# paninski-lab/deepgraphpose

Hardware: AMD Instinct MI355X
Metric: frames_per_sec (higher is better)
Workload: dtype f32

## Files before the change

### deepgraphpose_amd/csrc/dgp_chain.hip

```cpp
#include "dgp_internal.h"
#include "dgp_device.h"

#include <cstdio>
#include <cstdlib>
#include <type_traits>

namespace dgp {

typedef float floatx4 __attribute__((ext_vector_type(4)));
typedef __attribute__((address_space(3))) void lds_void;

__device__ __forceinline__ floatx4 mma16(const uint4& a, const uint4& b, floatx4 c) {
    return __builtin_amdgcn_mfma_f32_16x16x32_f16(__builtin_bit_cast(half8, a), __builtin_bit_cast(half8, b), c, 0, 0, 0);
}
__device__ __forceinline__ uint4 ld16nt(__amdgpu_buffer_rsrc_t r, unsigned voff, int soff) {
    return __builtin_bit_cast(uint4, __builtin_amdgcn_raw_buffer_load_b128(r, (int)voff, soff, 2));
}
__device__ __forceinline__ void st16nt(__amdgpu_buffer_rsrc_t r, const uint4& v, unsigned voff, int soff) {
    __builtin_amdgcn_raw_buffer_store_b128(__builtin_bit_cast(u32x4, v), r, (int)voff, soff, 2);
}
__device__ __forceinline__ uint4 ld16(__amdgpu_buffer_rsrc_t r, unsigned voff, int soff) {
    return __builtin_bit_cast(uint4, __builtin_amdgcn_raw_buffer_load_b128(r, (int)voff, soff, 0));
}
__device__ __forceinline__ void st16(__amdgpu_buffer_rsrc_t r, const uint4& v, unsigned voff, int soff) {
    __builtin_amdgcn_raw_buffer_store_b128(__builtin_bit_cast(u32x4, v), r, (int)voff, soff, 0);
}

#ifdef DGP_DIAG
__device__ unsigned long long g_unit_diag[16];
#define UD_STAMP(x)                                                                     \
    do {                                                                                \
        __builtin_amdgcn_sched_barrier(0);                                              \
        asm volatile("s_memtime %0\n\ts_waitcnt lgkmcnt(0)" : "=s"(x)::"memory");       \
        __builtin_amdgcn_sched_barrier(0);                                              \
    } while (0)
#define UD_PARAM , unsigned long long (&ud)[12]
#define UD_ARG , ud
#else
#define UD_STAMP(x)
#define UD_PARAM
#define UD_ARG
#endif

template <int RES, int RB, bool H1 = false>
__device__ __forceinline__ void chain_fetch_res(const ChainArgs& p, uint4 (&res)[RB][2], const unsigned (&roff)[RB],
                                                const __amdgpu_buffer_rsrc_t rs_s2, int jp) {
    if constexpr (RES != 0) {
#pragma unroll
        for (int rb = 0; rb < RB; ++rb) {
            if constexpr (H1) {
                res[rb][0] = (p.nt & 1) ? ld16nt(rs_s2, roff[rb], jp * 64) : ld16(rs_s2, roff[rb], jp * 64);
            } else if (p.nt & 1) {
                res[rb][0] = ld16nt(rs_s2, roff[rb], jp * 128);
                res[rb][1] = ld16nt(rs_s2, roff[rb], jp * 128 + 16);
            } else {
                res[rb][0] = ld16(rs_s2, roff[rb], jp * 128);
                res[rb][1] = ld16(rs_s2, roff[rb], jp * 128 + 16);
            }
        }
    }
}
template <int RES, int RB, int PD, bool H1 = false>
__device__ __forceinline__ void chain_prefetch(const ChainArgs& p, uint4 (&res)[PD][RB][2], const unsigned (&roff)[RB],
                                               const __amdgpu_buffer_rsrc_t rs_s2) {
#pragma unroll
    for (int u = 0; u < PD - 1; ++u) chain_fetch_res<RES, RB, H1>(p, res[u], roff, rs_s2, u);
}

template <int C, int C1, int CIN2, int RES, int RB, int NS, int PD, int CHUNK, int WR, bool H1 = false>
__device__ __forceinline__ void chain_tail(const ChainArgs& p, const uint4* ring, int& slot, const uint4 (&ph)[RB][(C + CIN2) / 32],
                                           const uint4 (&pl)[RB][(C + CIN2) / 32], const unsigned (&xoff)[RB], const unsigned (&roff)[RB],
                                           const unsigned (&r1off)[RB], const unsigned long long (&xkeep)[RB], const bool xwave,
                                           const __amdgpu_buffer_rsrc_t rs_s2, const __amdgpu_buffer_rsrc_t rs_xo,
                                           const __amdgpu_buffer_rsrc_t rs_r1, float& amax_x, float& amax_r1, const int lane,
                                           uint4 (&res)[PD][RB][2] UD_PARAM) {
#ifdef DGP_DIAG
    unsigned long long c0 = 0, c1 = 0, c2 = 0, c3 = 0, c4 = 0;
#endif
    constexpr int C4 = 4 * C, KS1 = (C + CIN2) / 32, NJP = C4 / 32, NCB = C1 / 16;
    constexpr int PL = H1 ? 1 : 2;
    constexpr int F1 = KS1 * 2 * PL, F2 = NCB * PL;
    static_assert(WR >= 2 && WR % 2 == 0, "weight fragments in flight: pairs share the ring");
    static_assert(NJP % PD == 0 && PD >= 2, "chunk loop is unrolled PD times");
    const int g = lane >> 4;
    floatx4 a2[RB][NCB];
#pragma unroll
    for (int rb = 0; rb < RB; ++rb)
#pragma unroll
        for (int cb = 0; cb < NCB; ++cb) a2[rb][cb] = floatx4{0.f, 0.f, 0.f, 0.f};
    auto fetch_res = [&](int jp, int buf) { chain_fetch_res<RES, RB, H1>(p, res[buf], roff, rs_s2, jp); };
    constexpr int CB = H1 ? 64 : 128;
    for (int jp0 = 0; jp0 < NJP; jp0 += PD) {
#pragma unroll
        for (int u = 0; u < PD; ++u) {
            const int jp = jp0 + u;
            if (jp + PD - 1 < NJP) fetch_res(jp + PD - 1, (u + PD - 1) % PD);
            UD_STAMP(c0);
            const uint4* Wc = ring + slot * (CHUNK / 16);
            const uint4* W = Wc + lane;
            floatx4 a1[RB][2];
#pragma unroll
            for (int rb = 0; rb < RB; ++rb) { a1[rb][0] = floatx4{0.f, 0.f, 0.f, 0.f}; a1[rb][1] = floatx4{0.f, 0.f, 0.f, 0.f}; }
            uint4 wq[WR];
#pragma unroll
            for (int f = 0; f < WR && f < F1 + F2; ++f) wq[f] = W[f * 64];
            __builtin_amdgcn_sched_barrier(0);
#pragma unroll
            for (int s = 0; s < KS1; ++s)
#pragma unroll
                for (int b = 0; b < 2; ++b) {
                    const int f0 = (s * 2 + b) * PL;
                    const uint4 wh = wq[f0 % WR], wl = wq[(f0 + PL - 1) % WR];
                    if constexpr (!H1) {
#pragma unroll
                    for (int rb = 0; rb < RB; ++rb) a1[rb][b] = mma16(wl, ph[rb][s], a1[rb][b]);
#pragma unroll
                    for (int rb = 0; rb < RB; ++rb) a1[rb][b] = mma16(wh, pl[rb][s], a1[rb][b]);
                    }
#pragma unroll
                    for (int rb = 0; rb < RB; ++rb) a1[rb][b] = mma16(wh, ph[rb][s], a1[rb][b]);
                    __builtin_amdgcn_sched_barrier(0);
                    if (f0 + WR < F1 + F2) wq[f0 % WR] = W[(f0 + WR) * 64];
                    if (PL == 2 && f0 + 1 + WR < F1 + F2) wq[(f0 + 1) % WR] = W[(f0 + 1 + WR) * 64];
                    __builtin_amdgcn_sched_barrier(0);
                }
            UD_STAMP(c1);
            const float4 sa = __builtin_bit_cast(float4, Wc[(F1 + F2) * 64 + 2 * g]), sb = __builtin_bit_cast(float4, Wc[(F1 + F2) * 64 + 2 * g + 1]);
            const float4 ba = __builtin_bit_cast(float4, Wc[(F1 + F2) * 64 + 8 + 2 * g]), bb = __builtin_bit_cast(float4, Wc[(F1 + F2) * 64 + 8 + 2 * g + 1]);
            const float sc[8] = {sa.x * p.post1, sa.y * p.post1, sa.z * p.post1, sa.w * p.post1,
                                 sb.x * p.post1, sb.y * p.post1, sb.z * p.post1, sb.w * p.post1};
            const float bi[8] = {ba.x, ba.y, ba.z, ba.w, bb.x, bb.y, bb.z, bb.w};
            uint4 xh[RB], xl[RB];
#pragma unroll
            for (int rb = 0; rb < RB; ++rb) {
                float o[8], r[8] = {0.f, 0.f, 0.f, 0.f, 0.f, 0.f, 0.f, 0.f};
                if constexpr (RES != 0) {
                    if constexpr (H1) h1_unpack8(res[u][rb][0], p.res_inv_scale, r);
                    else h2_unpack8(res[u][rb][0], res[u][rb][1], p.res_inv_scale, r);
                }
#pragma unroll
                for (int k = 0; k < 8; ++k) {
                    o[k] = a1[rb][k >> 2][k & 3] * sc[k] + bi[k] + r[k];
                    o[k] = fmaxf(o[k], 0.f);
                }
                if constexpr (H1) { xh[rb] = h1_pack8(o, p.xout_scale); xl[rb] = xh[rb]; }
                else h2_pack8(o, p.xout_scale, xh[rb], xl[rb]);
                if (xwave) {
                    const unsigned so = __builtin_amdgcn_inverse_ballot_w64(xkeep[rb]) ? xoff[rb] : OOB;
                    if (p.nt & 2) {
                        st16nt(rs_xo, xh[rb], so, jp * CB);
                        if constexpr (!H1) st16nt(rs_xo, xl[rb], so, jp * CB + 16);
                    } else {
                        st16(rs_xo, xh[rb], so, jp * CB);
                        if constexpr (!H1) st16(rs_xo, xl[rb], so, jp * CB + 16);
                    }
                }
                if (xoff[rb] != OOB) {
#pragma unroll
                    for (int k = 0; k < 8; ++k) amax_x = fmaxf(amax_x, o[k]);
                }
            }
            UD_STAMP(c2);
            __builtin_amdgcn_sched_barrier(0);
#pragma unroll
            for (int cb = 0; cb < NCB; ++cb) {
                const int f0 = F1 + cb * PL;
                const uint4 wh = wq[f0 % WR], wl = wq[(f0 + PL - 1) % WR];
                if constexpr (!H1) {
#pragma unroll
                for (int rb = 0; rb < RB; ++rb) a2[rb][cb] = mma16(wl, xh[rb], a2[rb][cb]);
#pragma unroll
                for (int rb = 0; rb < RB; ++rb) a2[rb][cb] = mma16(wh, xl[rb], a2[rb][cb]);
                }
#pragma unroll
                for (int rb = 0; rb < RB; ++rb) a2[rb][cb] = mma16(wh, xh[rb], a2[rb][cb]);
                __builtin_amdgcn_sched_barrier(0);
                if (f0 + WR < F1 + F2) wq[f0 % WR] = W[(f0 + WR) * 64];
                if (PL == 2 && f0 + 1 + WR < F1 + F2) wq[(f0 + 1) % WR] = W[(f0 + 1 + WR) * 64];
                __builtin_amdgcn_sched_barrier(0);
            }
            slot = slot + 1 == NS ? 0 : slot + 1;
            UD_STAMP(c3);
            asm volatile("s_waitcnt lgkmcnt(0)" ::: "memory");
            __builtin_amdgcn_s_barrier();
            UD_STAMP(c4);
#ifdef DGP_DIAG
            ud[4] += c1 - c0; ud[5] += c2 - c1; ud[6] += c3 - c2; ud[7] += c4 - c3;
#endif
        }
    }
    UD_STAMP(c0);
#pragma unroll
    for (int q = 0; q < NCB / 2; ++q) {
        const float4 s0 = *reinterpret_cast<const float4*>(p.sc1 + 32 * q + 8 * g), s1 = *reinterpret_cast<const float4*>(p.sc1 + 32 * q + 8 * g + 4);
        const float4 b0 = *reinterpret_cast<const float4*>(p.bi1 + 32 * q + 8 * g), b1 = *reinterpret_cast<const float4*>(p.bi1 + 32 * q + 8 * g + 4);
        const float sc[8] = {s0.x * p.post2, s0.y * p.post2, s0.z * p.post2, s0.w * p.post2,
                             s1.x * p.post2, s1.y * p.post2, s1.z * p.post2, s1.w * p.post2};
        const float bi[8] = {b0.x, b0.y, b0.z, b0.w, b1.x, b1.y, b1.z, b1.w};
#pragma unroll
        for (int rb = 0; rb < RB; ++rb) {
            float o[8];
#pragma unroll
            for (int k = 0; k < 8; ++k) o[k] = fmaxf(a2[rb][2 * q + (k >> 2)][k & 3] * sc[k] + bi[k], 0.f);
            if constexpr (H1) {
                st16(rs_r1, h1_pack8(o, p.r1_scale), r1off[rb], q * CB);
            } else {
            uint4 hi, lo;
            h2_pack8(o, p.r1_scale, hi, lo);
            st16(rs_r1, hi, r1off[rb], q * 128);
            st16(rs_r1, lo, r1off[rb], q * 128 + 16);
            }
            if (r1off[rb] != OOB) {
#pragma unroll
                for (int k = 0; k < 8; ++k) amax_r1 = fmaxf(amax_r1, o[k]);
            }
        }
    }
    UD_STAMP(c1);
#ifdef DGP_DIAG
    ud[8] += c1 - c0;
#endif
}

template <int C, int C1, int CIN2, int RES, int RB, int NCW, int NLW, int NS, int PD, int WR, bool H1 = false>
__global__ __launch_bounds__(64 * (NCW + NLW)) void chain_kernel(const ChainArgs p) {
    constexpr int C4 = 4 * C;
    constexpr int EB = H1 ? 2 : 4;
    constexpr int KSA = C / 32, KSB = CIN2 / 32, KS1 = KSA + KSB;
    constexpr int NJP = C4 / 32;
    constexpr int NCB = C1 / 16;
    constexpr int PL = H1 ? 1 : 2;
    constexpr int F1 = KS1 * 2 * PL, F2 = NCB * PL, NF = F1 + F2 + 1;
    constexpr int CHUNK = NF * 1024;
    constexpr int TILE = 16 * RB * NCW;
    static_assert(NJP % PD == 0 && PD >= 2, "chunk loop is unrolled PD times");
    static_assert(RES == 0 || CIN2 == 0, "residual or K-concatenated shortcut, not both");
    static_assert(NS == 2 || NS == 3, "ring protocols of the loader below");
    extern __shared__ __attribute__((aligned(16))) char smem[];
    const int lane = threadIdx.x & 63;
    const int wave = __builtin_amdgcn_readfirstlane(threadIdx.x >> 6);
    const int my_tiles = (p.ntiles - (int)blockIdx.x + (int)gridDim.x - 1) / (int)gridDim.x;
    const int total = my_tiles * NJP;

    if (wave >= NCW) {
        const int lw = wave - NCW;
        const __amdgpu_buffer_rsrc_t rs_w = __builtin_amdgcn_make_buffer_rsrc(const_cast<void*>(p.wfrag), 0, (int)p.w_bytes, 0x00020000);
        int jp = 0, slot = 0;
        auto run = [&](auto niw) {
            constexpr int NIW = decltype(niw)::value;
            auto issue = [&]() {
                char* dst = smem + slot * CHUNK;
                const int gbase = jp * CHUNK;
#pragma unroll
                for (int i = 0; i < NIW; ++i) {
                    const int f = lw + i * NLW;
                    __builtin_amdgcn_raw_ptr_buffer_load_lds(rs_w, (lds_void*)(dst + f * 1024), 16, lane * 16, gbase + f * 1024, 0, 0);
                }
                jp = jp + 1 == NJP ? 0 : jp + 1;
                slot = slot + 1 == NS ? 0 : slot + 1;
            };
            if constexpr (NS == 3) {
                if (total > 0) issue();
                if (total > 1) { issue(); asm volatile("s_waitcnt vmcnt(%0)" ::"n"(NIW) : "memory"); }
                else asm volatile("s_waitcnt vmcnt(0)" ::: "memory");
                __builtin_amdgcn_s_barrier();
                for (int it = 0; it < total; ++it) {
                    if (it + 2 < total) { issue(); asm volatile("s_waitcnt vmcnt(%0)" ::"n"(NIW) : "memory"); }
                    else asm volatile("s_waitcnt vmcnt(0)" ::: "memory");
                    __builtin_amdgcn_s_barrier();
                }
            } else {
                if (total > 0) issue();
                asm volatile("s_waitcnt vmcnt(0)" ::: "memory");
                __builtin_amdgcn_s_barrier();
                for (int it = 0; it < total; ++it) {
                    if (it + 1 < total) issue();
                    asm volatile("s_waitcnt vmcnt(0)" ::: "memory");
                    __builtin_amdgcn_s_barrier();
                }
            }
        };
        constexpr int NI_HI = (NF + NLW - 1) / NLW, NI_LO = NF / NLW;
        if (lw < NF % NLW || NI_HI == NI_LO) run(std::integral_constant<int, NI_HI>());
        else run(std::integral_constant<int, NI_LO>());
        return;
    }

    const int l15 = lane & 15, g = lane >> 4;
    const __amdgpu_buffer_rsrc_t rs_r2 = __builtin_amdgcn_make_buffer_rsrc(const_cast<void*>(p.r2), 0, (int)p.r2_bytes, 0x00020000);
    const __amdgpu_buffer_rsrc_t rs_s2 = __builtin_amdgcn_make_buffer_rsrc(const_cast<void*>(p.src2 ? p.src2 : p.r2), 0,
                                                                            p.src2 ? (int)p.src2_bytes : 0, 0x00020000);
    const __amdgpu_buffer_rsrc_t rs_xo = __builtin_amdgcn_make_buffer_rsrc(p.xout, 0, (int)p.xout_bytes, 0x00020000);
    const __amdgpu_buffer_rsrc_t rs_r1 = __builtin_amdgcn_make_buffer_rsrc(p.r1out, 0, (int)p.r1_bytes, 0x00020000);
    const uint4* ring = reinterpret_cast<const uint4*>(smem);
    int slot = 0;
    float amax_x = 0.f, amax_r1 = 0.f;
    __builtin_amdgcn_s_barrier();
    for (int t = blockIdx.x; t < p.ntiles; t += gridDim.x) {
        unsigned xoff[RB], roff[RB], r1off[RB];
        unsigned long long xkeep[RB];
#pragma unroll
        for (int rb = 0; rb < RB; ++rb) xkeep[rb] = ~0ull;
        if (p.xkeep == 2) {
            unsigned HoWo = (unsigned)p.HoWo, Wo = (unsigned)p.Wo;
            asm volatile("" : "+s"(HoWo), "+s"(Wo));
#pragma unroll
            for (int rb = 0; rb < RB; ++rb) {
                const unsigned m = (unsigned)(t * TILE + (wave * RB + rb) * 16 + l15);
                const unsigned rem = m % HoWo, ho = rem / Wo, wo = rem - ho * Wo;
                xkeep[rb] = __builtin_amdgcn_ballot_w64(((ho | wo) & 1) == 0);
            }
        }
        uint4 ph[RB][KS1], pl[RB][KS1];
#pragma unroll
        for (int rb = 0; rb < RB; ++rb) {
            const int m = t * TILE + (wave * RB + rb) * 16 + l15;
            const bool ok = m < p.M;
            xoff[rb] = ok ? (unsigned)m * (unsigned)(C4 * EB) + (unsigned)(g * 8 * EB) : OOB;
            r1off[rb] = ok ? (unsigned)m * (unsigned)(C1 * EB) + (unsigned)(g * 8 * EB) : OOB;
            if (RES == 2) {
                const int n = m / p.HoWo, rem = m - n * p.HoWo, ho = rem / p.Wo, wo = rem - ho * p.Wo;
                roff[rb] = ok ? (unsigned)((n * p.res_H + 2 * ho) * p.res_W + 2 * wo) * (unsigned)(C4 * EB) + (unsigned)(g * 8 * EB) : OOB;
            } else roff[rb] = xoff[rb];
            const unsigned aoff = ok ? (unsigned)m * (unsigned)(C * EB) + (unsigned)(g * 8 * EB) : OOB;
#pragma unroll
            for (int s = 0; s < KSA; ++s) {
                ph[rb][s] = ld16(rs_r2, aoff, s * 32 * EB);
                if constexpr (H1) pl[rb][s] = ph[rb][s]; else pl[rb][s] = ld16(rs_r2, aoff, s * 128 + 16);
            }
            if constexpr (KSB > 0) {
                const unsigned boff = ok ? (unsigned)m * (unsigned)(CIN2 * EB) + (unsigned)(g * 8 * EB) : OOB;
#pragma unroll
                for (int s = 0; s < KSB; ++s) {
                    ph[rb][KSA + s] = ld16(rs_s2, boff, s * 32 * EB);
                    if constexpr (H1) pl[rb][KSA + s] = ph[rb][KSA + s]; else pl[rb][KSA + s] = ld16(rs_s2, boff, s * 128 + 16);
                }
            }
        }
        uint4 res[PD][RB][2];
        chain_prefetch<RES, RB, PD, H1>(p, res, roff, rs_s2);
#ifdef DGP_DIAG
        unsigned long long ud[12] = {0};
#endif
        chain_tail<C, C1, CIN2, RES, RB, NS, PD, CHUNK, WR, H1>(p, ring, slot, ph, pl, xoff, roff, r1off, xkeep, true, rs_s2, rs_xo, rs_r1, amax_x, amax_r1, lane, res UD_ARG);
#ifdef DGP_DIAG
        if (wave == 0 && lane == 0) {
            for (int i = 4; i < 9; ++i) atomicAdd(&g_unit_diag[i], ud[i]);
            atomicAdd(&g_unit_diag[9], 1ull);
        }
#endif
    }
    if (p.xout_absmax) track_absmax(p.xout_absmax, amax_x, lane, (int)(blockIdx.x * 8u + (unsigned)wave));
    if (p.r1_absmax) track_absmax(p.r1_absmax, amax_r1, lane, (int)(blockIdx.x * 8u + (unsigned)wave) + 97);
}

template <int C, int C1, int CIN2, int RES, int NCW, int NLW, int PD, int WR, int HWV = 1, bool H1 = false>
__global__ __launch_bounds__(64 * (NCW + NLW + HWV)) void unit_kernel(const ChainArgs p) {
    constexpr int NS = 3;
    constexpr int TH = NCW, TW = 16, HW = TW + 2, HPIX = (TH + 2) * HW;
    constexpr int EB = H1 ? 2 : 4;
    constexpr int PIXB = C * EB;
    constexpr int PPI = 1024 / PIXB;
    static_assert(C == 64, "one pixel of R1 = 16 (H1: 8) slots of 16 bytes (the bank swizzle)");
    constexpr int NHI = (HPIX * PIXB + 1023) / 1024;
    constexpr int HALO_BYTES = NHI * 1024;
    static_assert(NLW == 1 || NLW == 2 || NLW == 4, "one, two or four weight-loader waves");
    static_assert(HWV == 0 || HWV == 1, "at most one halo wave");
    constexpr int NHW = HWV ? 1 : NLW;
    constexpr int C4 = 4 * C, KS1 = (C + CIN2) / 32, NJP = C4 / 32, NCB = C1 / 16;
    constexpr int PL = H1 ? 1 : 2;
    constexpr int NFJ = (KS1 * 2 + NCB) * PL + 1;
    constexpr int KS2 = C / 32, NCB2 = C / 16, NF2 = KS2 * NCB2 * PL + 1;
    constexpr int NFMAX = NFJ > NF2 ? NFJ : NF2, CHUNK = NFMAX * 1024;
    constexpr int STEPS = 9 + NJP;
    constexpr int HSTEPS = HWV ? NJP - 1 : NJP;
    constexpr int HPP = (NHI + HSTEPS - 1) / HSTEPS;
    extern __shared__ __attribute__((aligned(16))) char smem[];
    char* halo = smem;
    char* ringb = smem + HALO_BYTES;
    const int lane = threadIdx.x & 63;
    const int wave = __builtin_amdgcn_readfirstlane(threadIdx.x >> 6);
    const int G = (int)gridDim.x, b = (int)blockIdx.x;
    const int vwg = (G & 7) == 0 ? (b & 7) * (G >> 3) + (b >> 3) : b;
    const int my_tiles = vwg < p.ntiles ? (p.ntiles - vwg + G - 1) / G : 0;
    const int total = my_tiles * STEPS;
    const int tpf = p.TY * p.TX;

    if (wave >= NCW) {
        auto halo_issue = [&](int tile, int i0, int i1, int hl) {
            const __amdgpu_buffer_rsrc_t rs_in = __builtin_amdgcn_make_buffer_rsrc(const_cast<void*>(p.r1in), 0, (int)p.r1in_bytes, 0x00020000);
            const int f = tile / tpf, rem = tile - f * tpf, ty = rem / p.TX, tx = rem - ty * p.TX;
            for (int i = i0 + hl; i < i1; i += NHW) {
                const int hp = PPI * i + (H1 ? (lane >> 3) : (lane >> 4));
                const int hy = (hp * 57) >> 10, hx = hp - HW * hy;
                const int gy = ty * TH - 1 + hy, gx = tx * TW - 1 + hx;
                const bool ok = hp < HPIX && (unsigned)gy < (unsigned)p.H && (unsigned)gx < (unsigned)p.W;
                const unsigned cell = H1 ? (unsigned)((lane & 7) ^ ((hp >> 1) & 7)) : (unsigned)((lane & 15) ^ (hp & 15));
                const unsigned off = ok ? (unsigned)((f * p.H + gy) * p.W + gx) * (unsigned)PIXB + (cell << 4) : OOB;
                __builtin_amdgcn_raw_ptr_buffer_load_lds(rs_in, (lds_void*)(halo + i * 1024), 16, (int)off, 0, 0, 0);
            }
        };
        auto halo_step = [&](int cur_st, int tile, int hl) {
            if (cur_st >= 9 && tile + G < p.ntiles) {
                const int i0 = (cur_st - 9) * HPP, i1 = i0 + HPP < NHI ? i0 + HPP : NHI;
                halo_issue(tile + G, i0, i1, hl);
            }
        };
        const int lw_rt = wave - NCW;
        if (HWV && lw_rt == NLW) {
            if (total > 0) halo_issue(vwg, 0, NHI, 0);
            asm volatile("s_waitcnt vmcnt(0)" ::: "memory");
            __builtin_amdgcn_s_barrier();
            int cur_st = 0, tile = vwg;
            for (int it = 0; it < total; ++it) {
                halo_step(cur_st, tile, 0);
                if (cur_st == STEPS - 1) asm volatile("s_waitcnt vmcnt(0)" ::: "memory");
                __builtin_amdgcn_s_barrier();
                if (++cur_st == STEPS) { cur_st = 0; tile += G; }
            }
            return;
        }
        auto loader = [&](auto lw_c) {
        constexpr int lw = decltype(lw_c)::value;
        const __amdgpu_buffer_rsrc_t rs_w = __builtin_amdgcn_make_buffer_rsrc(const_cast<void*>(p.wfrag), 0, (int)p.w_bytes, 0x00020000);
        int st = 0, slot = 0;
        constexpr int N2 = lw < NF2 % NLW ? (NF2 + NLW - 1) / NLW : NF2 / NLW, NJ = lw < NFJ % NLW ? (NFJ + NLW - 1) / NLW : NFJ / NLW;
        auto issue = [&]() {
            char* dst = ringb + slot * CHUNK;
            const int st2 = st, stj = st - 9;
            if (st < 9) {
#pragma unroll
                for (int k = 0; k < N2; ++k)
                    __builtin_amdgcn_raw_ptr_buffer_load_lds(rs_w, (lds_void*)(dst + (lw + k * NLW) * 1024), 16, lane * 16, st2 * (NF2 * 1024) + (lw + k * NLW) * 1024, 0, 0);
            } else {
#pragma unroll
                for (int k = 0; k < NJ; ++k)
                    __builtin_amdgcn_raw_ptr_buffer_load_lds(rs_w, (lds_void*)(dst + (lw + k * NLW) * 1024), 16, lane * 16,
                                                             9 * (NF2 * 1024) + stj * (NFJ * 1024) + (lw + k * NLW) * 1024, 0, 0);
            }
            const bool was_conv2 = st < 9;
            st = st + 1 == STEPS ? 0 : st + 1;
            slot = slot + 1 == NS ? 0 : slot + 1;
            return was_conv2;
        };
        auto wait_all_but_newest = [&](bool conv2_chunk) {
            if (conv2_chunk) asm volatile("s_waitcnt vmcnt(%0)" ::"n"(N2) : "memory");
            else asm volatile("s_waitcnt vmcnt(%0)" ::"n"(NJ) : "memory");
        };
        if (total > 0) {
            if (!HWV) halo_issue(vwg, 0, NHI, lw);
            issue();
            wait_all_but_newest(issue());
        }
        __builtin_amdgcn_s_barrier();
        int cur_st = 0, tile = vwg;
#ifdef DGP_DIAG
        unsigned long long l0 = 0, l1 = 0, l2 = 0, l3 = 0, ul[3] = {0, 0, 0}, ul3 = 0;
#endif
        for (int it = 0; it < total; ++it) {
            UD_STAMP(l0);
            if (!HWV) halo_step(cur_st, tile, lw);
#ifdef DGP_DIAG
            bool c2_ = false;
            if (it + 2 < total) c2_ = issue();
            UD_STAMP(l1);
            if (it + 2 < total) wait_all_but_newest(c2_);
            else asm volatile("s_waitcnt vmcnt(0)" ::: "memory");
            UD_STAMP(l2);
#else
            if (it + 2 < total) wait_all_but_newest(issue());
            else asm volatile("s_waitcnt vmcnt(0)" ::: "memory");
#endif
            __builtin_amdgcn_s_barrier();
            UD_STAMP(l3);
#ifdef DGP_DIAG
            if (cur_st < 9) ul[0] += l1 - l0; else ul3 += l1 - l0;
            ul[1] += l2 - l1; ul[2] += l3 - l2;
#endif
            if (++cur_st == STEPS) { cur_st = 0; tile += G; }
        }
#ifdef DGP_DIAG
        if (lw == 0 && lane == 0) {
            atomicAdd(&g_unit_diag[12], ul[0]); atomicAdd(&g_unit_diag[13], ul[1]); atomicAdd(&g_unit_diag[14], ul[2]); atomicAdd(&g_unit_diag[11], ul3);
            atomicAdd(&g_unit_diag[15], (unsigned long long)total);
        }
#endif
        };
        if (lw_rt == 0) loader(std::integral_constant<int, 0>());
        else if (NLW > 1 && lw_rt == 1) loader(std::integral_constant<int, (NLW > 1 ? 1 : 0)>());
        else if (NLW > 2 && lw_rt == 2) loader(std::integral_constant<int, (NLW > 2 ? 2 : 0)>());
        else if (NLW > 3) loader(std::integral_constant<int, (NLW > 3 ? 3 : 0)>());
        return;
    }

    const int l15 = lane & 15, g = lane >> 4;
    const __amdgpu_buffer_rsrc_t rs_s2 = __builtin_amdgcn_make_buffer_rsrc(const_cast<void*>(p.src2), 0, (int)p.src2_bytes, 0x00020000);
    const __amdgpu_buffer_rsrc_t rs_xo = __builtin_amdgcn_make_buffer_rsrc(p.xout, 0, (int)p.xout_bytes, 0x00020000);
    const __amdgpu_buffer_rsrc_t rs_r1 = __builtin_amdgcn_make_buffer_rsrc(p.r1out, 0, (int)p.r1_bytes, 0x00020000);
    const uint4* ring = reinterpret_cast<const uint4*>(ringb);
    int slot = 0;
    float amax_x = 0.f, amax_r1 = 0.f, amax_r2 = 0.f;
    __builtin_amdgcn_s_barrier();
#ifdef DGP_DIAG
    unsigned long long ud[12] = {0}, u0 = 0, u1 = 0, u2 = 0, ubeg = 0, uend = 0;
    UD_STAMP(ubeg);
#endif
    for (int tile = vwg; tile < p.ntiles; tile += G) {
        UD_STAMP(u0);
        const int f = tile / tpf, rem = tile - f * tpf, ty = rem / p.TX, tx = rem - ty * p.TX;
        const int y = ty * TH + wave, x = tx * TW + l15;
        const bool ok = y < p.H && x < p.W;
        const int m = (f * p.H + y) * p.W + x;
        unsigned xoff[1], roff[1], r1off[1];
        xoff[0] = ok ? (unsigned)m * (unsigned)(C4 * EB) + (unsigned)(g * 8 * EB) : OOB;
        roff[0] = xoff[0];
        r1off[0] = ok ? (unsigned)m * (unsigned)(C1 * EB) + (unsigned)(g * 8 * EB) : OOB;
        const bool xsub = p.xkeep == 2;
        const bool xwave = !(xsub && (y & 1));
        const unsigned long long xkeep[1] = {xsub ? __builtin_amdgcn_ballot_w64((x & 1) == 0) : ~0ull};
        uint4 ph[1][KS1], pl[1][KS1];
        if constexpr (CIN2 > 0) {
            const unsigned boff = ok ? (unsigned)m * (unsigned)(CIN2 * EB) + (unsigned)(g * 8 * EB) : OOB;
#pragma unroll
            for (int s = 0; s < CIN2 / 32; ++s) {
                ph[0][KS2 + s] = ld16(rs_s2, boff, s * 32 * EB);
                if constexpr (H1) pl[0][KS2 + s] = ph[0][KS2 + s]; else pl[0][KS2 + s] = ld16(rs_s2, boff, s * 128 + 16);
            }
        }
        uint4 res[PD][1][2];
        chain_prefetch<RES, 1, PD, H1>(p, res, roff, rs_s2);
        floatx4 acc[NCB2];
#pragma unroll
        for (int cb = 0; cb < NCB2; ++cb) acc[cb] = floatx4{0.f, 0.f, 0.f, 0.f};
        uint4 aff[KS2][4];
        UD_STAMP(u1);
#ifdef DGP_DIAG
        ud[3] += u1 - u0;
#endif
#pragma unroll
        for (int t = 0; t < 9; ++t) {
            UD_STAMP(u0);
            const uint4* Wc = ring + slot * (CHUNK / 16);
            const uint4* W = Wc + lane;
            const int hp = (wave + t / 3) * HW + l15 + t % 3;
            const char* hrow = halo + hp * PIXB;
            const int sw = H1 ? ((hp >> 1) & 7) : (hp & 15);
            uint4 ah[KS2], al[KS2];
#pragma unroll
            for (int ks = 0; ks < KS2; ++ks) {
                if constexpr (H1) {
                    ah[ks] = *reinterpret_cast<const uint4*>(hrow + (((4 * ks + g) ^ sw) << 4));
                    al[ks] = ah[ks];
                } else {
                const int sl = 2 * (4 * ks + g);
                ah[ks] = *reinterpret_cast<const uint4*>(hrow + ((sl ^ sw) << 4));
                al[ks] = *reinterpret_cast<const uint4*>(hrow + (((sl + 1) ^ sw) << 4));
                }
            }
            constexpr int NW2 = KS2 * NCB2 * PL;
            uint4 wq[WR];
#pragma unroll
            for (int f = 0; f < WR && f < NW2; ++f) wq[f] = W[f * 64];
            __builtin_amdgcn_sched_barrier(0);
#pragma unroll
            for (int ks = 0; ks < KS2; ++ks) {
#pragma unroll
                for (int cb = 0; cb < NCB2; ++cb) {
                    const int f0 = (ks * NCB2 + cb) * PL;
                    const uint4 wh = wq[f0 % WR], wl = wq[(f0 + PL - 1) % WR];
                    if constexpr (!H1) {
                    acc[cb] = mma16(wl, ah[ks], acc[cb]);
                    acc[cb] = mma16(wh, al[ks], acc[cb]);
                    }
                    acc[cb] = mma16(wh, ah[ks], acc[cb]);
                    __builtin_amdgcn_sched_barrier(0);
                    if (f0 + WR < NW2) wq[f0 % WR] = W[(f0 + WR) * 64];
                    if (PL == 2 && f0 + 1 + WR < NW2) wq[(f0 + 1) % WR] = W[(f0 + 1 + WR) * 64];
                    __builtin_amdgcn_sched_barrier(0);
                }
            }
            if (t == 8) {
#pragma unroll
                for (int q = 0; q < KS2; ++q) {
                    aff[q][0] = Wc[(NF2 - 1) * 64 + 8 * q + 2 * g]; aff[q][1] = Wc[(NF2 - 1) * 64 + 8 * q + 2 * g + 1];
                    aff[q][2] = Wc[(NF2 - 1) * 64 + 16 + 8 * q + 2 * g]; aff[q][3] = Wc[(NF2 - 1) * 64 + 16 + 8 * q + 2 * g + 1];
                }
            }
            slot = slot + 1 == NS ? 0 : slot + 1;
            UD_STAMP(u1);
            asm volatile("s_waitcnt lgkmcnt(0)" ::: "memory");
            __builtin_amdgcn_s_barrier();
            UD_STAMP(u2);
#ifdef DGP_DIAG
            ud[0] += u1 - u0; ud[1] += u2 - u1;
#endif
        }
        UD_STAMP(u0);
#pragma unroll
        for (int q = 0; q < KS2; ++q) {
            const float4 sa = __builtin_bit_cast(float4, aff[q][0]), sb = __builtin_bit_cast(float4, aff[q][1]);
            const float4 ba = __builtin_bit_cast(float4, aff[q][2]), bb = __builtin_bit_cast(float4, aff[q][3]);
            const float sc[8] = {sa.x * p.post0, sa.y * p.post0, sa.z * p.post0, sa.w * p.post0, sb.x * p.post0, sb.y * p.post0, sb.z * p.post0, sb.w * p.post0};
            const float bi[8] = {ba.x, ba.y, ba.z, ba.w, bb.x, bb.y, bb.z, bb.w};
            float o[8];
#pragma unroll
            for (int k = 0; k < 8; ++k) o[k] = fmaxf(acc[2 * q + (k >> 2)][k & 3] * sc[k] + bi[k], 0.f);
            if constexpr (H1) { ph[0][q] = h1_pack8(o, p.r2_scale); pl[0][q] = ph[0][q]; }
            else h2_pack8(o, p.r2_scale, ph[0][q], pl[0][q]);
            if (ok) {
#pragma unroll
                for (int k = 0; k < 8; ++k) amax_r2 = fmaxf(amax_r2, o[k]);
            }
        }
        UD_STAMP(u1);
#ifdef DGP_DIAG
        ud[2] += u1 - u0; ud[9] += 1;
#endif
        chain_tail<C, C1, CIN2, RES, 1, NS, PD, CHUNK, WR, H1>(p, ring, slot, ph, pl, xoff, roff, r1off, xkeep, xwave, rs_s2, rs_xo, rs_r1, amax_x, amax_r1, lane, res UD_ARG);
    }
#ifdef DGP_DIAG
    UD_STAMP(uend);
    ud[10] = uend - ubeg;
    if (wave == 0 && lane == 0)
        for (int i = 0; i < 11; ++i) atomicAdd(&g_unit_diag[i], ud[i]);
#endif
    if (p.xout_absmax) track_absmax(p.xout_absmax, amax_x, lane, (int)(blockIdx.x * 8u + (unsigned)wave));
    if (p.r1_absmax) track_absmax(p.r1_absmax, amax_r1, lane, (int)(blockIdx.x * 8u + (unsigned)wave) + 97);
    if (p.r2_absmax) track_absmax(p.r2_absmax, amax_r2, lane, (int)(blockIdx.x * 8u + (unsigned)wave) + 41);
}

__global__ __launch_bounds__(256) void chain_pack_kernel(const float4* __restrict__ src, int n_chunks, int f1_pairs, int f2_pairs,
                                                         float s1, float s2, uint4* __restrict__ out, int planes) {
    const int pairs = f1_pairs + f2_pairs;
    const int nf = planes * pairs + 1;
    const long long src_chunk = (long long)pairs * 128 + 64;
    const long long total = (long long)n_chunks * (pairs + 1) * 64;
    for (long long i = (long long)blockIdx.x * blockDim.x + threadIdx.x; i < total; i += (long long)gridDim.x * blockDim.x) {
        const int ln = (int)(i & 63);
        const long long fp = i >> 6;
        const int ch = (int)(fp / (pairs + 1)), pr = (int)(fp % (pairs + 1));
        uint4* o = out + ((long long)ch * nf + planes * pr) * 64 + ln;
        if (pr == pairs) {
            o[0] = __builtin_bit_cast(uint4, src[ch * src_chunk + (long long)pairs * 128 + ln]);
            continue;
        }
        const float4* sp = src + ch * src_chunk + (long long)pr * 128 + ln * 2;
        uint2 h0, l0, h1, l1;
        const float sc = pr < f1_pairs ? s1 : s2;
        split2_f16(sp[0], sc, h0, l0);
        split2_f16(sp[1], sc, h1, l1);
        o[0] = make_uint4(h0.x, h0.y, h1.x, h1.y);
        if (planes == 2) o[64] = make_uint4(l0.x, l0.y, l1.x, l1.y);
    }
}

hipError_t launch_chain_pack(const float* src, int n_chunks, int f1_pairs, int f2_pairs, float s1, float s2, void* out, hipStream_t s, int planes) {
    const long long total = (long long)n_chunks * (f1_pairs + f2_pairs + 1) * 64;
    long long blocks = (total + 255) / 256;
    if (blocks > 4096) blocks = 4096;
    hipLaunchKernelGGL(chain_pack_kernel, dim3((unsigned)blocks), dim3(256), 0, s, reinterpret_cast<const float4*>(src), n_chunks, f1_pairs,
                       f2_pairs, s1, s2, reinterpret_cast<uint4*>(out), planes);
    return hipGetLastError();
}

namespace {

template <int C, int C1, int CIN2, int RES, int RB, int NCW, int NLW, int PD, int NS = 3, int WR = 4, bool H1 = false>
hipError_t launch_chain_t(const ChainArgs& a0, hipStream_t s) {
    constexpr int NF = ((C + CIN2) / 32 * 2 + C1 / 16) * (H1 ? 1 : 2) + 1;
    constexpr int LDS = NS * NF * 1024;
    static_assert(LDS <= 160 * 1024, "ring does not fit the LDS");
    constexpr auto kern = chain_kernel<C, C1, CIN2, RES, RB, NCW, NLW, NS, PD, WR, H1>;
    hipError_t e = ensure_dynamic_lds<kern>(LDS);
    if (e != hipSuccess) return e;
    const DeviceFacts dev = device_facts();
    static int wgs_per_cu[16] = {};
    if (!wgs_per_cu[dev.slot]) {
        int occ = 0;
        e = hipOccupancyMaxActiveBlocksPerMultiprocessor(&occ, kern, 64 * (NCW + NLW), LDS);
        if (e != hipSuccess) return e;
        static const int force = dgp_tune("DGP_CHAIN_WGS", 0);
        wgs_per_cu[dev.slot] = force > 0 ? force : (occ < 1 ? 1 : occ);
    }
    ChainArgs a = a0;
    static const int nt_env = dgp_tune("DGP_CHAIN_NT", 0);
    a.nt = nt_env;
    constexpr int TILE = 16 * RB * NCW;
    a.ntiles = (a.M + TILE - 1) / TILE;
    int grid = dev.n_cu * wgs_per_cu[dev.slot];
    if (grid > a.ntiles) grid = a.ntiles;
    if (grid < 1) return hipSuccess;
#ifdef DGP_DIAG
    unsigned long long hz[16] = {0};
    (void)hipMemcpyToSymbol(HIP_SYMBOL(g_unit_diag), hz, sizeof(hz));
#endif
    hipLaunchKernelGGL(kern, dim3((unsigned)grid), dim3(64 * (NCW + NLW)), LDS, s, a);
#ifdef DGP_DIAG
    (void)hipStreamSynchronize(s);
    (void)hipMemcpyFromSymbol(hz, HIP_SYMBOL(g_unit_diag), sizeof(hz));
    const double nt = (double)hz[9] > 0 ? (double)hz[9] : 1.0, ns = (double)hz[15] > 0 ? (double)hz[15] : 1.0;
    printf("[diag chain C %d C1 %d CIN2 %d] grid %d tiles %d (%.1f per workgroup) | compute wave 0, cycles per TILE: prologue %.0f | conv2: 9 x (work %.0f + barrier %.0f) "
           "epilogue %.0f | chain: %d x (conv3 %.0f + epilogue %.0f + conv1 %.0f + barrier %.0f) conv1 epilogue %.0f | tile loop %.0f per tile | "
           "loader wave 0, cycles per STEP: issue %.0f (conv2 steps) / %.0f (pointwise steps), vmcnt wait %.0f, barrier %.0f\n", C, C1, CIN2, grid, a.ntiles, (double)a.ntiles / grid,
           hz[3] / nt, hz[0] / nt / 9.0, hz[1] / nt / 9.0, hz[2] / nt, 4 * C / 32, hz[4] / nt / (4 * C / 32), hz[5] / nt / (4 * C / 32), hz[6] / nt / (4 * C / 32),
           hz[7] / nt / (4 * C / 32), hz[8] / nt, hz[10] * (double)grid / nt / grid, hz[12] / (ns * 9.0 / (9.0 + 4 * C / 32)), hz[11] / (ns * (4 * C / 32) / (9.0 + 4 * C / 32)), hz[13] / ns, hz[14] / ns);
#endif
    return hipGetLastError();
}

template <int C, int C1, int CIN2, int RES, int NCW, int NLW, int PD, int WR = 4, int HWV = 1, bool H1 = false>
hipError_t launch_unit_t(const ChainArgs& a0, int N, hipStream_t s) {
    constexpr int NFJ = ((C + CIN2) / 32 * 2 + C1 / 16) * (H1 ? 1 : 2) + 1, NF2 = (C / 32) * (C / 16) * (H1 ? 1 : 2) + 1, NFMAX = NFJ > NF2 ? NFJ : NF2;
    constexpr int LDS = ((NCW + 2) * 18 * C * (H1 ? 2 : 4) + 1023) / 1024 * 1024 + 3 * NFMAX * 1024;
    static_assert(LDS <= 160 * 1024, "halo tile + ring do not fit the LDS");
    constexpr auto kern = unit_kernel<C, C1, CIN2, RES, NCW, NLW, PD, WR, HWV, H1>;
    hipError_t e = ensure_dynamic_lds<kern>(LDS);
    if (e != hipSuccess) return e;
    const DeviceFacts dev = device_facts();
    static int wgs_per_cu[16] = {};
    if (!wgs_per_cu[dev.slot]) {
        int occ = 0;
        e = hipOccupancyMaxActiveBlocksPerMultiprocessor(&occ, kern, 64 * (NCW + NLW + HWV), LDS);
        if (e != hipSuccess) return e;
        static const int force = dgp_tune("DGP_CHAIN_WGS", 0);
        wgs_per_cu[dev.slot] = force > 0 ? force : (occ < 1 ? 1 : occ);
    }
    ChainArgs a = a0;
    static const int nt_env = dgp_tune("DGP_CHAIN_NT", 0);
    a.nt = nt_env;
    a.TY = (a.H + NCW - 1) / NCW; a.TX = (a.W + 15) / 16;
    a.ntiles = N * a.TY * a.TX;
    int grid = dev.n_cu * wgs_per_cu[dev.slot];
    if (grid > a.ntiles) grid = a.ntiles;
    if (grid < 1) return hipSuccess;
#ifdef DGP_DIAG
    unsigned long long hz[16] = {0};
    (void)hipMemcpyToSymbol(HIP_SYMBOL(g_unit_diag), hz, sizeof(hz));
#endif
    hipLaunchKernelGGL(kern, dim3((unsigned)grid), dim3(64 * (NCW + NLW + HWV)), LDS, s, a);
#ifdef DGP_DIAG
    (void)hipStreamSynchronize(s);
    (void)hipMemcpyFromSymbol(hz, HIP_SYMBOL(g_unit_diag), sizeof(hz));
    const double nt = (double)hz[9] > 0 ? (double)hz[9] : 1.0, ns = (double)hz[15] > 0 ? (double)hz[15] : 1.0;
    printf("[diag unit  C %d C1 %d CIN2 %d] grid %d tiles %d (%.1f per workgroup) | compute wave 0, cycles per TILE: prologue %.0f | conv2: 9 x (work %.0f + barrier %.0f) "
           "epilogue %.0f | chain: %d x (conv3 %.0f + epilogue %.0f + conv1 %.0f + barrier %.0f) conv1 epilogue %.0f | tile loop %.0f per tile | "
           "loader wave 0, cycles per STEP: issue %.0f (conv2 steps) / %.0f (pointwise steps), vmcnt wait %.0f, barrier %.0f\n", C, C1, CIN2, grid, a.ntiles, (double)a.ntiles / grid,
           hz[3] / nt, hz[0] / nt / 9.0, hz[1] / nt / 9.0, hz[2] / nt, 4 * C / 32, hz[4] / nt / (4 * C / 32), hz[5] / nt / (4 * C / 32), hz[6] / nt / (4 * C / 32),
           hz[7] / nt / (4 * C / 32), hz[8] / nt, hz[10] * (double)grid / nt / grid, hz[12] / (ns * 9.0 / (9.0 + 4 * C / 32)), hz[11] / (ns * (4 * C / 32) / (9.0 + 4 * C / 32)), hz[13] / ns, hz[14] / ns);
#endif
    return hipGetLastError();
}

}

bool chain_supported(int C, int C1, int CIN2, int res) {
    if (C == 64 && C1 == 64 && CIN2 == 0 && res == 1) return true;
    if (C == 64 && C1 == 64 && CIN2 == 64 && res == 0) return true;
    if (C == 64 && C1 == 128 && CIN2 == 0 && res == 2) return true;
    if (C == 128 && C1 == 128 && CIN2 == 0 && res == 1) return true;
    if (C == 128 && C1 == 256 && CIN2 == 0 && res == 2) return true;
    if (C == 256 && C1 == 256 && CIN2 == 0 && res == 1) return true;
    return false;
}

bool unit_supported(int C, int C1, int CIN2, int res) {
    return C == 64 && C1 == 64 && ((CIN2 == 0 && res == 1) || (CIN2 == 64 && res == 0));
}

hipError_t launch_unit(const ChainArgs& a, int N, int C, int C1, int CIN2, int res, hipStream_t s) {
    static const int cfg = dgp_tune("DGP_UNIT_CFG", 0);
    if (C == 64 && C1 == 64 && CIN2 == 0 && res == 1) {
        if (cfg == 1) return launch_unit_t<64, 64, 0, 1, 8, 4, 2, 4, 0>(a, N, s);
        if (cfg == 2) return launch_unit_t<64, 64, 0, 1, 10, 2, 2, 4, 0>(a, N, s);
        if (cfg == 3) return launch_unit_t<64, 64, 0, 1, 8, 2, 2, 4, 1>(a, N, s);
        if (a.h1) return launch_unit_t<64, 64, 0, 1, 8, 4, 2, 4, 1, true>(a, N, s);
        return launch_unit_t<64, 64, 0, 1, 8, 2, 2, 4, 0>(a, N, s);
    }
    if (C == 64 && C1 == 64 && CIN2 == 64 && res == 0) {
        if (cfg == 1) return launch_unit_t<64, 64, 64, 0, 8, 4, 2, 8, 0>(a, N, s);
        if (cfg == 2) return launch_unit_t<64, 64, 64, 0, 10, 2, 2, 8, 0>(a, N, s);
        if (cfg == 3) return launch_unit_t<64, 64, 64, 0, 8, 2, 2, 8, 0>(a, N, s);
        if (a.h1) return launch_unit_t<64, 64, 64, 0, 8, 2, 2, 8, 1, true>(a, N, s);
        return launch_unit_t<64, 64, 64, 0, 8, 2, 2, 8, 1>(a, N, s);
    }
    return hipErrorInvalidValue;
}

int chain_frags_per_chunk(int C, int C1, int CIN2, int planes) { return ((C + CIN2) / 32 * 2 + C1 / 16) * planes + 1; }

const char* chain_kernel_name(int C, int C1, int CIN2, int res) {
    static thread_local char buf[64];
    snprintf(buf, sizeof buf, "chain_c%d_n%d_%s", C, C1, res == 0 ? "sc" : (res == 2 ? "s2" : "id"));
    (void)CIN2;
    return buf;
}

hipError_t launch_chain(const ChainArgs& a, int C, int C1, int CIN2, int res, hipStream_t s) {
    static const int cfg = dgp_tune("DGP_CHAIN_CFG", 0);
    if (C == 64 && C1 == 64 && CIN2 == 0 && res == 1) {
        if (cfg == 1) return launch_chain_t<64, 64, 0, 1, 2, 5, 1, 4>(a, s);
        if (cfg == 2) return launch_chain_t<64, 64, 0, 1, 2, 4, 1, 2>(a, s);
        if (cfg == 3) return launch_chain_t<64, 64, 0, 1, 1, 11, 1, 4>(a, s);
        if (cfg == 4) return launch_chain_t<64, 64, 0, 1, 1, 8, 2, 4>(a, s);
        if (cfg == 5) return launch_chain_t<64, 64, 0, 1, 1, 8, 4, 4>(a, s);
        if (a.h1) return launch_chain_t<64, 64, 0, 1, 1, 8, 1, 4, 3, 4, true>(a, s);
        return launch_chain_t<64, 64, 0, 1, 1, 8, 1, 4>(a, s);
    }
    if (C == 64 && C1 == 64 && CIN2 == 64 && res == 0) {
        if (cfg == 1) return launch_chain_t<64, 64, 64, 0, 2, 5, 1, 2>(a, s);
        if (cfg == 4) return launch_chain_t<64, 64, 64, 0, 1, 8, 2, 2>(a, s);
        if (cfg == 5) return launch_chain_t<64, 64, 64, 0, 1, 8, 4, 2>(a, s);
        if (a.h1) return launch_chain_t<64, 64, 64, 0, 1, 8, 1, 2, 3, 4, true>(a, s);
        return launch_chain_t<64, 64, 64, 0, 1, 8, 1, 2>(a, s);
    }
    if (C == 64 && C1 == 128 && CIN2 == 0 && res == 2) {
        if (cfg == 1) return launch_chain_t<64, 128, 0, 2, 2, 5, 1, 4>(a, s);
        if (cfg == 4) return launch_chain_t<64, 128, 0, 2, 1, 8, 2, 4>(a, s);
        if (cfg == 5) return launch_chain_t<64, 128, 0, 2, 1, 8, 4, 4>(a, s);
        if (a.h1) return launch_chain_t<64, 128, 0, 2, 1, 8, 1, 4, 3, 4, true>(a, s);
        return launch_chain_t<64, 128, 0, 2, 1, 8, 1, 4>(a, s);
    }
    if (C == 128 && C1 == 128 && CIN2 == 0 && res == 1) {
        if (cfg == 1) return launch_chain_t<128, 128, 0, 1, 1, 8, 2, 4, 3, 4>(a, s);
        if (cfg == 2) return launch_chain_t<128, 128, 0, 1, 1, 8, 2, 2, 3, 8>(a, s);
        if (cfg == 3) return launch_chain_t<128, 128, 0, 1, 1, 6, 2, 2, 3, 8>(a, s);
        if (cfg == 4 || cfg == 5) return launch_chain_t<128, 128, 0, 1, 1, 8, 4, 2, 3, 4>(a, s);
        if (a.h1) return launch_chain_t<128, 128, 0, 1, 1, 8, 2, 2, 3, 4, true>(a, s);
        return launch_chain_t<128, 128, 0, 1, 1, 8, 2, 2, 3, 4>(a, s);
    }
    if (C == 128 && C1 == 256 && CIN2 == 0 && res == 2) {
        if (a.h1) return launch_chain_t<128, 256, 0, 2, 1, 6, 2, 4, 3, 4, true>(a, s);
        return launch_chain_t<128, 256, 0, 2, 1, 6, 2, 4>(a, s);
    }
    if (C == 256 && C1 == 256 && CIN2 == 0 && res == 1) {
        if (cfg == 1) return launch_chain_t<256, 256, 0, 1, 1, 4, 2, 2, 2, 8>(a, s);
        if (cfg == 2) return launch_chain_t<256, 256, 0, 1, 1, 6, 2, 2, 2, 8>(a, s);
        if (cfg == 3) return launch_chain_t<256, 256, 0, 1, 1, 5, 2, 2, 2, 4>(a, s);
        if (a.h1) return launch_chain_t<256, 256, 0, 1, 1, 5, 2, 2, 2, 8, true>(a, s);
        return launch_chain_t<256, 256, 0, 1, 1, 5, 2, 2, 2, 8>(a, s);
    }
    return hipErrorInvalidValue;
}

}
```

Measured before the change: 4782.

## Let compute waves self-load weight chunks into LDS via buffer-to-LDS DMA

Adds a self-DMA mode where the compute waves issue buffer_load ... lds pieces for the next weight chunk, interleaved between conv3 MFMA groups, instead of dedicating loader waves (NLW=0). Residual prefetch is moved after the DMA pieces, and vmcnt waits before the barrier are adjusted to count the outstanding stores and residual loads. The default 256x256 residual config switches to 8 compute waves, no loader waves and two ring slots, and the old config moves to cfg 6. This frees loader wavefronts and overlaps weight staging with MFMA work, at the risk of fragile hand-counted waitcnt logic, a shallower ring, and the loss of non-temporal stores on this path.

```diff
diff --git a/deepgraphpose_amd/csrc/dgp_chain.hip b/deepgraphpose_amd/csrc/dgp_chain.hip
--- a/deepgraphpose_amd/csrc/dgp_chain.hip
+++ b/deepgraphpose_amd/csrc/dgp_chain.hip
@@ -67,13 +67,69 @@
     for (int u = 0; u < PD - 1; ++u) chain_fetch_res<RES, RB, H1>(p, res[u], roff, rs_s2, u);
 }
 
-template <int C, int C1, int CIN2, int RES, int RB, int NS, int PD, int CHUNK, int WR, bool H1 = false>
+struct ChainNoDma {
+    static constexpr bool on = false;
+};
+__device__ __forceinline__ void chain_dma_piece(const u32x4& rsrc, unsigned lds_addr, unsigned voff, int soff) {
+    unsigned keep;
+    asm volatile("s_mov_b32 %0, m0\n\ts_mov_b32 m0, %1\n\ts_nop 0\n\tbuffer_load_dwordx4 %2, %3, %4 offen lds\n\ts_mov_b32 m0, %0"
+                 : "=&s"(keep)
+                 : "s"(lds_addr), "v"(voff), "s"(rsrc), "s"(soff)
+                 : "memory");
+}
+template <int NF, int NCW, int NS, int NJP>
+struct ChainSelfDma {
+    static constexpr bool on = true;
+    static constexpr int NPIECES = (NF + NCW - 1) / NCW;
+    static constexpr int CHUNK = NF * 1024;
+    u32x4 rs_w;
+    unsigned ring;
+    int wave;
+    unsigned voff;
+    int jp, slot, left;
+    __device__ __forceinline__ void init(const void* wfrag, unsigned bytes, const char* smem, int wave_, int lane, int total) {
+        const unsigned long long a = (unsigned long long)(size_t)wfrag;
+        rs_w = u32x4{(unsigned)a, (unsigned)(a >> 32) & 0xffffu, bytes, 0x00020000u};
+        ring = (unsigned)(size_t)smem; wave = wave_; voff = (unsigned)lane * 16u;
+        jp = 0; slot = 0; left = total;
+    }
+    __device__ __forceinline__ void piece(int i) const {
+        if (left <= 0) return;
+        if (i * NCW + NCW > NF && wave >= NF % NCW) return;
+        const unsigned dst = ring + (unsigned)(slot * CHUNK + wave * 1024);
+        const int gbase = jp * CHUNK + wave * 1024;
+        chain_dma_piece(rs_w, dst + i * (NCW * 1024), voff, gbase + i * (NCW * 1024));
+    }
+    __device__ __forceinline__ void advance() {
+        if (left <= 0) return;
+        jp = jp + 1 == NJP ? 0 : jp + 1;
+        slot = slot + 1 == NS ? 0 : slot + 1;
+        --left;
+    }
+    __device__ __forceinline__ void issue() {
+#pragma unroll
+        for (int i = 0; i < NPIECES; ++i) piece(i);
+        advance();
+    }
+};
+template <class DMA>
+constexpr int chain_dma_pieces() {
+    if constexpr (DMA::on) return DMA::NPIECES; else return 0;
+}
+template <int N>
+__device__ __forceinline__ void chain_wait_vm() {
+    static_assert(N >= 0 && N < 16, "s_waitcnt immediate: vmcnt[3:0], expcnt and lgkmcnt left at their maxima");
+    asm volatile("s_waitcnt vmcnt(%0)" ::"n"(N) : "memory");
+    __builtin_amdgcn_s_waitcnt(0x0F70 | N);
+}
+
+template <int C, int C1, int CIN2, int RES, int RB, int NS, int PD, int CHUNK, int WR, bool H1 = false, class DMA = ChainNoDma>
 __device__ __forceinline__ void chain_tail(const ChainArgs& p, const uint4* ring, int& slot, const uint4 (&ph)[RB][(C + CIN2) / 32],
                                            const uint4 (&pl)[RB][(C + CIN2) / 32], const unsigned (&xoff)[RB], const unsigned (&roff)[RB],
                                            const unsigned (&r1off)[RB], const unsigned long long (&xkeep)[RB], const bool xwave,
                                            const __amdgpu_buffer_rsrc_t rs_s2, const __amdgpu_buffer_rsrc_t rs_xo,
                                            const __amdgpu_buffer_rsrc_t rs_r1, float& amax_x, float& amax_r1, const int lane,
-                                           uint4 (&res)[PD][RB][2] UD_PARAM) {
+                                           uint4 (&res)[PD][RB][2], DMA& dma UD_PARAM) {
 #ifdef DGP_DIAG
     unsigned long long c0 = 0, c1 = 0, c2 = 0, c3 = 0, c4 = 0;
 #endif
@@ -94,7 +150,8 @@
 #pragma unroll
         for (int u = 0; u < PD; ++u) {
             const int jp = jp0 + u;
-            if (jp + PD - 1 < NJP) fetch_res(jp + PD - 1, (u + PD - 1) % PD);
+            const bool fetched = jp + PD - 1 < NJP;
+            if (!DMA::on && fetched) fetch_res(jp + PD - 1, (u + PD - 1) % PD);
             UD_STAMP(c0);
             const uint4* Wc = ring + slot * (CHUNK / 16);
             const uint4* W = Wc + lane;
@@ -123,7 +180,14 @@
                     if (f0 + WR < F1 + F2) wq[f0 % WR] = W[(f0 + WR) * 64];
                     if (PL == 2 && f0 + 1 + WR < F1 + F2) wq[(f0 + 1) % WR] = W[(f0 + 1 + WR) * 64];
                     __builtin_amdgcn_sched_barrier(0);
-                }
+                    if constexpr (DMA::on) {
+                        static_assert(chain_dma_pieces<DMA>() <= KS1 * 2, "a piece per MFMA group of conv3");
+                        if (s * 2 + b < chain_dma_pieces<DMA>()) dma.piece(s * 2 + b);
+                        if (s * 2 + b == chain_dma_pieces<DMA>() - 1 && fetched) fetch_res(jp + PD - 1, (u + PD - 1) % PD);
+                        __builtin_amdgcn_sched_barrier(0);
+                    }
+                }
+            if constexpr (DMA::on) dma.advance();
             UD_STAMP(c1);
             const float4 sa = __builtin_bit_cast(float4, Wc[(F1 + F2) * 64 + 2 * g]), sb = __builtin_bit_cast(float4, Wc[(F1 + F2) * 64 + 2 * g + 1]);
             const float4 ba = __builtin_bit_cast(float4, Wc[(F1 + F2) * 64 + 8 + 2 * g]), bb = __builtin_bit_cast(float4, Wc[(F1 + F2) * 64 + 8 + 2 * g + 1]);
@@ -147,7 +211,7 @@
                 else h2_pack8(o, p.xout_scale, xh[rb], xl[rb]);
                 if (xwave) {
                     const unsigned so = __builtin_amdgcn_inverse_ballot_w64(xkeep[rb]) ? xoff[rb] : OOB;
-                    if (p.nt & 2) {
+                    if (!DMA::on && (p.nt & 2)) {
                         st16nt(rs_xo, xh[rb], so, jp * CB);
                         if constexpr (!H1) st16nt(rs_xo, xl[rb], so, jp * CB + 16);
                     } else {
@@ -182,6 +246,13 @@
             slot = slot + 1 == NS ? 0 : slot + 1;
             UD_STAMP(c3);
             asm volatile("s_waitcnt lgkmcnt(0)" ::: "memory");
+            if constexpr (DMA::on) {
+                constexpr int NX = RB * (H1 ? 1 : 2);
+                constexpr int NR = RES != 0 ? RB * (H1 ? 1 : 2) : 0;
+                if (NR > 0 && fetched) { if (xwave) chain_wait_vm<NX + NR>(); else chain_wait_vm<NR>(); }
+                else if (xwave) chain_wait_vm<NX>();
+                else chain_wait_vm<0>();
+            }
             __builtin_amdgcn_s_barrier();
             UD_STAMP(c4);
 #ifdef DGP_DIAG
@@ -236,12 +307,14 @@
     static_assert(NJP % PD == 0 && PD >= 2, "chunk loop is unrolled PD times");
     static_assert(RES == 0 || CIN2 == 0, "residual or K-concatenated shortcut, not both");
     static_assert(NS == 2 || NS == 3, "ring protocols of the loader below");
+    static_assert(NLW > 0 || NS == 2, "self-loading mode: one chunk ahead, two slots");
     extern __shared__ __attribute__((aligned(16))) char smem[];
     const int lane = threadIdx.x & 63;
     const int wave = __builtin_amdgcn_readfirstlane(threadIdx.x >> 6);
     const int my_tiles = (p.ntiles - (int)blockIdx.x + (int)gridDim.x - 1) / (int)gridDim.x;
     const int total = my_tiles * NJP;
 
+    if constexpr (NLW > 0)
     if (wave >= NCW) {
         const int lw = wave - NCW;
         const __amdgpu_buffer_rsrc_t rs_w = __builtin_amdgcn_make_buffer_rsrc(const_cast<void*>(p.wfrag), 0, (int)p.w_bytes, 0x00020000);
@@ -280,8 +353,9 @@
                 }
             }
         };
-        constexpr int NI_HI = (NF + NLW - 1) / NLW, NI_LO = NF / NLW;
-        if (lw < NF % NLW || NI_HI == NI_LO) run(std::integral_constant<int, NI_HI>());
+        constexpr int NLD = NLW > 0 ? NLW : 1;
+        constexpr int NI_HI = (NF + NLD - 1) / NLD, NI_LO = NF / NLD;
+        if (lw < NF % NLD || NI_HI == NI_LO) run(std::integral_constant<int, NI_HI>());
         else run(std::integral_constant<int, NI_LO>());
         return;
     }
@@ -295,6 +369,13 @@
     const uint4* ring = reinterpret_cast<const uint4*>(smem);
     int slot = 0;
     float amax_x = 0.f, amax_r1 = 0.f;
+    using Dma = std::conditional_t<NLW == 0, ChainSelfDma<NF, NCW, NS, NJP>, ChainNoDma>;
+    Dma dma;
+    if constexpr (NLW == 0) {
+        dma.init(p.wfrag, (unsigned)p.w_bytes, smem, wave, lane, total);
+        dma.issue();
+        asm volatile("s_waitcnt vmcnt(0)" ::: "memory");
+    }
     __builtin_amdgcn_s_barrier();
     for (int t = blockIdx.x; t < p.ntiles; t += gridDim.x) {
         unsigned xoff[RB], roff[RB], r1off[RB];
@@ -342,7 +423,8 @@
 #ifdef DGP_DIAG
         unsigned long long ud[12] = {0};
 #endif
-        chain_tail<C, C1, CIN2, RES, RB, NS, PD, CHUNK, WR, H1>(p, ring, slot, ph, pl, xoff, roff, r1off, xkeep, true, rs_s2, rs_xo, rs_r1, amax_x, amax_r1, lane, res UD_ARG);
+        if constexpr (NLW == 0) __builtin_amdgcn_s_waitcnt(0x0F70);
+        chain_tail<C, C1, CIN2, RES, RB, NS, PD, CHUNK, WR, H1, Dma>(p, ring, slot, ph, pl, xoff, roff, r1off, xkeep, true, rs_s2, rs_xo, rs_r1, amax_x, amax_r1, lane, res, dma UD_ARG);
 #ifdef DGP_DIAG
         if (wave == 0 && lane == 0) {
             for (int i = 4; i < 9; ++i) atomicAdd(&g_unit_diag[i], ud[i]);
@@ -616,7 +698,8 @@
 #ifdef DGP_DIAG
         ud[2] += u1 - u0; ud[9] += 1;
 #endif
-        chain_tail<C, C1, CIN2, RES, 1, NS, PD, CHUNK, WR, H1>(p, ring, slot, ph, pl, xoff, roff, r1off, xkeep, xwave, rs_s2, rs_xo, rs_r1, amax_x, amax_r1, lane, res UD_ARG);
+        ChainNoDma nodma;
+        chain_tail<C, C1, CIN2, RES, 1, NS, PD, CHUNK, WR, H1>(p, ring, slot, ph, pl, xoff, roff, r1off, xkeep, xwave, rs_s2, rs_xo, rs_r1, amax_x, amax_r1, lane, res, nodma UD_ARG);
     }
 #ifdef DGP_DIAG
     UD_STAMP(uend);
@@ -836,8 +919,12 @@
         if (cfg == 1) return launch_chain_t<256, 256, 0, 1, 1, 4, 2, 2, 2, 8>(a, s);
         if (cfg == 2) return launch_chain_t<256, 256, 0, 1, 1, 6, 2, 2, 2, 8>(a, s);
         if (cfg == 3) return launch_chain_t<256, 256, 0, 1, 1, 5, 2, 2, 2, 4>(a, s);
-        if (a.h1) return launch_chain_t<256, 256, 0, 1, 1, 5, 2, 2, 2, 8, true>(a, s);
-        return launch_chain_t<256, 256, 0, 1, 1, 5, 2, 2, 2, 8>(a, s);
+        if (cfg == 6) {
+            if (a.h1) return launch_chain_t<256, 256, 0, 1, 1, 5, 2, 2, 2, 8, true>(a, s);
+            return launch_chain_t<256, 256, 0, 1, 1, 5, 2, 2, 2, 8>(a, s);
+        }
+        if (a.h1) return launch_chain_t<256, 256, 0, 1, 1, 8, 0, 4, 2, 4, true>(a, s);
+        return launch_chain_t<256, 256, 0, 1, 1, 8, 0, 4, 2, 4>(a, s);
     }
     return hipErrorInvalidValue;
 }
```

Result: no change. 4774 (median of 2 runs) (-0.2%).
